# hvasbath/beat

Measured on AMD Instinct MI355X. Metric: SMC chain-steps/s (FFI seismic gfstacking 400 patches x 64 targets x 4096 samples), higher is better.
Workload: dtype f64; 1 GPU; BASELINE configs[2]: FFI seismic gfstacking, 400 patches x 64 targets x 4096 samples, library (64,400,3,25,4096) f64 = 62.9 GB in HBM, nearest_neighbor, covariance scalar; population SURVEY 8(d): nucleation U over the 20x20 fault, time 0; chains_per_gpu=512, global_chains=512, parallelism=chains sharded over 1 GPU(s), library replicated

## Files before the change

### beat_amd/_lib.py

```python
import ctypes as C
import os

import numpy as np

_HERE = os.path.dirname(os.path.abspath(__file__))
LIB_PATH = os.environ.get("BEATAMD_LIB") or os.path.join(_HERE, "libbeat_amd.so")

NEAREST_NEIGHBOR, MULTILINEAR = 0, 1
W_SCALAR, W_DENSE = 0, 1
INTERPOLATIONS = {"nearest_neighbor": NEAREST_NEIGHBOR, "multilinear": MULTILINEAR}

OK, EINVAL, EHIP, EINDEX, ENOMEM, ENAN, ENOTPSD, EBADCOV, EOUTSIDE = 0, -1, -2, -3, -4, -5, -6, -7, -8
ABI_VERSION = 120


class BeatAmdError(RuntimeError):
    pass


class FfiLayout(C.Structure):
    _fields_ = [
        ("nparams", C.c_int64),
        ("nvar", C.c_int32),
        ("slip_off", C.c_int64 * 4),
# ... 33 lines not shown
    "beatamd_geo_stack_all_batch": [_vp, _i32, _i64, _vp, _i32, _vp],
    "beatamd_weights_create": [_vp, _i32, _i64, _i64, _vp, _vp, _pi32],
    "beatamd_weights_update": [_vp, _i32, _i32, _i64, _vp, _vp],
    "beatamd_weights_destroy": [_vp, _i32],
    "beatamd_weights_band": [_vp, _i32, _pi64],
    "beatamd_weights_band_info": [_vp, _i32, _pi64, C.POINTER(_f64)],
    "beatamd_mvn_chol_logp_batch": [_vp, _i32, _i64, _vp, _vp, _vp],
    "beatamd_laplacian_create": [_vp, _i64, _vp, _f64, _pi32],
    "beatamd_laplacian_destroy": [_vp, _i32],
    "beatamd_laplacian_logp_batch": [_vp, _i32, _i64, _i64, _vp, _vp, _vp],
    "beatamd_ffi_model_create": [_vp, C.POINTER(FfiLayout), _i32, _vp, _vp, _vp, _pi32],
    "beatamd_ffi_model_add_wavemap": [_vp, _i32, _vp, _vp, _i32, _vp, _vp, _i32],
    "beatamd_ffi_model_add_geodetic": [_vp, _i32, _vp, _vp, _vp, _i32, _vp, _vp, _vp],
    "beatamd_ffi_model_add_geodetic_geometry": [_vp, _i32, _i32, _vp, _vp, _vp, _i64, _vp, _vp, _vp, _f64,
                                                _vp, _vp, _i32, _vp, _vp, _vp],
    "beatamd_ffi_model_add_geodetic_corrections": [_vp, _i32, _i32, _vp, _vp, _vp, _vp, _vp],
    "beatamd_ffi_model_set_laplacian": [_vp, _i32, _i32],
    "beatamd_ffi_model_nllk": [_vp, _i32, _pi64],
    "beatamd_ffi_model_destroy": [_vp, _i32],
    "beatamd_ffi_logp_batch": [_vp, _i32, _i64, _vp, _vp],
    "beatamd_ffi_synthetics_batch": [_vp, _i32, _i32, _i64, _vp, _i32, _vp],
    "beatamd_ffi_astep_batch": [_vp, _i32, _i64, _vp, _vp, _vp, _vp, _vp, _vp, _vp, _f64, _vp],
    "beatamd_autocovariance_batch": [_vp, _i64, _i64, _vp, _vp, _vp],
    "beatamd_scaled_toeplitz_batch": [_vp, _i64, _i64, _vp, _vp, _vp],
    "beatamd_ffi_astep_batch_betas": [_vp, _i32, _i64, _vp, _vp, _vp, _vp, _vp, _vp, _vp, _vp, _vp],
    "beatamd_ffi_mstep_batch": [_vp, _i32, _i64, _vp, _vp, _vp, _i64, _i32, _i32, C.c_uint64, C.c_uint32, _i64,
                                _vp, _vp, _vp, _f64, _vp, _vp, _vp, _vp],
    "beatamd_ctx_last_kernel": [_vp, C.c_char_p, _i64],
    "beatamd_ctx_gf_group_stats": [_vp, _pi64, C.POINTER(_f64), _pi64, _pi64],
    "beatamd_ctx_gf_plan": [_vp, C.c_char_p, _i64, C.POINTER(_f64), _pi64],
    "beatamd_ctx_gf_tune_log": [_vp, C.c_char_p, _i64],
    "beatamd_gf_patch_ranges": [_i64, _i64, _i64, C.c_int32],
    "beatamd_seis_gflib_set_split_targets": [_vp, _i32, _i64],
    "beatamd_ctx_reload_knobs": [_vp],
    "beatamd_ctx_gf_chain_groups": [_vp, _i64, _vp, _vp, _i64, _vp],
    "beatamd_smc_calc_beta": [_vp, _i64, _vp, _i64, _f64, _f64, C.POINTER(_f64), _vp],
    "beatamd_smc_stage_weights": [_vp, _i64, _vp, _i64, _f64, _vp],
    "beatamd_smc_resample": [_vp, _i64, _vp, _f64, _vp],
    "beatamd_smc_population_factor": [_vp, _i64, _i64, _vp, _vp, _vp],
    "beatamd_proposal_draw": [_vp, _i64, _i64, _i64, _vp, C.c_uint64, C.c_uint32, _i64, _i32, _vp, _vp],
    "beatamd_proposal_draw_univariate": [_vp, _i64, _i64, _i32, _vp, C.c_uint64, C.c_uint32, _i64, _vp, _vp],
    "beatamd_gather_rows": [_vp, _i64, _i64, _vp, _i64, _vp, _vp],
    "beatamd_metropolis_tune": [_vp, _i64, _vp, _vp, _i32],
    "beatamd_ffi_model_nterm": [_vp, _i32, _pi64],
    "beatamd_ffi_llks_batch": [_vp, _i32, _i64, _vp, _vp],
    "beatamd_hyper_model_create": [_vp, _i64, _i64, _vp, _vp, _vp, _vp, _i32, _vp, _pi32],
    "beatamd_hyper_model_destroy": [_vp, _i32],
    "beatamd_hyper_logp_batch": [_vp, _i32, _i64, _vp, _vp, _vp],
    "beatamd_hyper_chain_batch": [_vp, _i32, _i64, _i64, _vp, _vp, _vp, _vp, _vp, _vp, _vp, _i32, _vp, C.c_uint64,
                                  C.c_uint32, _i64, _i32, _i32, _i32, _vp, _vp],
    "beatamd_wset_quad_batch": [_vp, _i32, _i64, _vp, _vp],
    "beatamd_ffi_obs_quads": [_vp, _i32, _vp],
    "beatamd_ffi_variance_reductions_batch": [_vp, _i32, _i64, _vp, _vp],
    "beatamd_ffi_geo_residuals_batch": [_vp, _i32, _i64, _vp, _i32, _vp],
    "beatamd_standardize_batch": [_vp, _i32, _vp, _i64, _i64, _i64, _vp, _vp, _vp],
    "beatamd_ensemble_moments_update": [_vp, _i64, _i64, _vp, _vp, _i64],
    "beatamd_ensemble_moments_finish": [_vp, _i64, _vp, _i64, _vp, _vp, _vp, _vp],
    "beatamd_trace_density_update": [_vp, _i64, _i64, _i64, _vp, _vp, _f64, _vp, _i64, _i64, _f64, _vp],
    "beatamd_like_assemble": [_vp, _i64, _i64, _i64, _vp, _vp, _vp, _i64, _i64, _i64, _i64, _i32, _vp, _vp],
    "beatamd_metropolis_propose": [_vp, _i64, _i64, _vp, _vp, _vp, _vp, _vp, _vp, _vp],
    "beatamd_metropolis_accept": [_vp, _i64, _i64, _i64, _vp, _vp, _vp, _vp, _vp, _vp, _f64, _vp, _vp],
    "beatamd_whiten_rows": [_vp, _vp, _i64, _i64, _vp],
    "beatamd_whiten_rows_batch": [_vp, _vp, _i64, _i64, _i64, _vp],
    "beatamd_chol_inverse_batch": [_vp, _i64, _i64, _vp, _vp, _vp],
    "beatamd_chol_inverse_batch_flags": [_vp, _i64, _i64, _vp, _vp, _vp, _vp],
    "beatamd_whitening_ratio_batch": [_vp, _i64, _i64, _vp, _vp, _vp],
# ... 77 lines not shown
```

### beat_amd/csrc/capi.cpp

```cpp
#include "model.hpp"

using namespace beatamd;

namespace {

template <class T>
int32_t add_obj(std::vector<std::unique_ptr<T>> &v, std::unique_ptr<T> o)
{
    for (size_t i = 0; i < v.size(); i++)
        if (!v[i]) {
            v[i] = std::move(o);
            return (int32_t)i;
        }
    v.push_back(std::move(o));
    return (int32_t)v.size() - 1;
}

template <class T>
int host_copy(beatamd_ctx *ctx, const T *p, size_t n, std::vector<T> &out)
{
    out.resize(n);
    if (n == 0) return BEATAMD_OK;
    if (is_device_ptr(p)) {
        BA_HIP(hipMemcpyAsync(out.data(), p, n * sizeof(T), hipMemcpyDeviceToHost, ctx->stream));
// ... 1148 lines not shown
    *row_bytes = (int64_t)((double)tot * ctx->gs_trep) * ctx->gs_N * 8 * ctx->gs_nvar;
    return BEATAMD_OK;
}

int beatamd_ctx_gf_plan(beatamd_ctx *ctx, char *buf, int64_t buflen, double *mean_passes, int64_t *max_passes)
{
    ENTER(ctx);
    BA_CHECK(buf && buflen > 0, BEATAMD_EINVAL, "gf_plan: bad argument");
    snprintf(buf, (size_t)buflen, "%s", ctx->gf_plan);
    if (mean_passes) *mean_passes = ctx->gs_ngtp ? 1.0 : 0.0;
    if (max_passes) *max_passes = ctx->gs_ngtp ? 1 : 0;
    if (!ctx->gs_has_passes || ctx->gs_ngtp == 0 || (!mean_passes && !max_passes)) return BEATAMD_OK;
    int64_t tot = 0, mx = 0;
    BA_TRY(gs_counters(ctx, 1, &tot, &mx));
    if (mean_passes) *mean_passes = (double)tot / (double)ctx->gs_ngtp;
    if (max_passes) *max_passes = mx;
    return BEATAMD_OK;
}

int beatamd_ctx_gf_tune_log(beatamd_ctx *ctx, char *buf, int64_t buflen)
{
    ENTER(ctx);
    BA_CHECK(buf && buflen > 0, BEATAMD_EINVAL, "gf_tune_log: bad argument");
    snprintf(buf, (size_t)buflen, "%s", ctx->gf_tune_log);
    return BEATAMD_OK;
}

int32_t beatamd_gf_patch_ranges(int64_t ntargets, int64_t npatches, int64_t nsamples, int32_t num_cu)
{
    if (ntargets <= 0 || npatches <= 0 || nsamples <= 0) return 1;
    return (int32_t)gf_patch_ranges(ntargets, npatches, nsamples, num_cu > 0 ? num_cu : 256);
}

int beatamd_ctx_gf_chain_groups(beatamd_ctx *ctx, int64_t C, const double *key0, const double *key1,
                                int64_t chains_per_group, uint32_t *members)
{
    ENTER(ctx);
    BA_CHECK(C > 0 && key0 && key1 && members && chains_per_group > 0, BEATAMD_EINVAL, "gf_chain_groups: bad argument");
    const int64_t ngroups = (C + chains_per_group - 1) / chains_per_group;
    const ChainVec key[2] = {ChainVec{key0, 1, 0}, ChainVec{key1, 1, 0}};
    const uint32_t *m = nullptr;
    BA_TRY(launch_chain_members(ctx, C, key, chains_per_group, ngroups, &m));
    BA_CHECK(m != nullptr, BEATAMD_EINVAL, "gf_chain_groups: groups of more than 8192 chains are not cut");
    BA_HIP(hipStreamSynchronize(ctx->stream));
    BA_HIP(hipMemcpy(members, m, (size_t)(ngroups * chains_per_group) * sizeof(uint32_t), hipMemcpyDeviceToHost));
    return BEATAMD_OK;
}

int beatamd_smc_calc_beta(beatamd_ctx *ctx, int64_t C, const double *likelihoods, int64_t stride,
                          double beta, double coef_variation, double *beta_new, double *weights)
{
    ENTER(ctx);
    BA_CHECK(likelihoods && beta_new && weights && C > 0 && stride > 0, BEATAMD_EINVAL,
             "smc_calc_beta: bad argument");
    Staging st(ctx);
    const double *d_l;
    double *d_w, *d_out;
    BA_TRY(st.in(likelihoods, (size_t)((C - 1) * stride + 1), &d_l));
    BA_TRY(st.out(weights, (size_t)C, &d_w));
    BA_TRY(ctx->scratch(SL_STAGE2, 8, &d_out));
    BA_TRY(launch_smc_calc_beta(ctx, C, d_l, stride, beta, coef_variation, 0, 0.0, d_out, d_w));
    double out[2];
    BA_HIP(hipMemcpyAsync(out, d_out, sizeof(out), hipMemcpyDeviceToHost, ctx->stream));
    BA_TRY(st.finish());
    BA_HIP(hipStreamSynchronize(ctx->stream));
    *beta_new = out[0];
// ... 383 lines not shown
```

### beat_amd/csrc/gfshared.hip

```cpp
#include "kernels.hpp"
#include "misfit.hpp"

namespace beatamd {

constexpr int GS_NT_MAX = 64;
constexpr int GS_NTHINT_DEFAULT = 1;
constexpr int GS_WS_DEFAULT = 1;

struct GroupTabArgs {
    int nrow, nvar, CG;
    int64_t C, T, P, DS;
    const uint32_t *rowoff;
    const double *fac;
    ChainVec slips[4];
    int ucap, ustride;
    uint32_t *urows;
    uint32_t *uent;
    int nissue;
    int windowed;
    int depth;
    uint32_t *ucount;
    uint32_t *umax;
    uint16_t *slot;
    double *w;
// ... 1237 lines not shown
{
    __shared__ uint32_t wsum[WS_CG / 64];
    const int tid = threadIdx.x;
    const int lane = tid & 63, wv = tid >> 6;
    const int64_t pos = (int64_t)blockIdx.x * WS_CG + tid;
    const uint32_t c = order ? order[pos] : (pos < C ? (uint32_t)pos : 0xffffffffu);
    const bool on = c != 0xffffffffu && (int64_t)c < C && active[c] != 0;
    const uint64_t m = __ballot(on);
    if (lane == 0) wsum[wv] = (uint32_t)__popcll(m);
    __syncthreads();
    uint32_t before = 0, total = 0;
    for (int q = 0; q < WS_CG / 64; q++) {
        const uint32_t x = wsum[q];
        if (q < wv) before += x;
        total += x;
    }
    uint32_t *o = out + (int64_t)blockIdx.x * WS_CG;
    if (on) o[before + (uint32_t)__popcll(m & ((1ull << lane) - 1ull))] = c;
    if ((uint32_t)tid >= total) o[tid] = 0xffffffffu;
}

constexpr int64_t WS_MAP_MAX = 16384;
template <int FILL, int MAP>
__global__ void __launch_bounds__(WS_CG) k_ws_tables(WsTabArgs a)
{
    extern __shared__ __attribute__((aligned(16))) uint16_t rowmap[];
    __shared__ __attribute__((aligned(16))) uint32_t vals[WS_CG];
    __shared__ __attribute__((aligned(16))) uint32_t firstv[WS_CG];
    __shared__ uint32_t lst[WS_CG];
    __shared__ uint32_t gm[WS_CG];
    __shared__ uint16_t slt[WS_CG];
    __shared__ uint8_t rk2i[WS_MAXPASS][128];
    __shared__ uint32_t wsum[WS_CG / 64 + 1];
    const int tid = threadIdx.x;
    const int lane = tid & 63, wv = tid >> 6;
    const int64_t gtp = xcd_items8(blockIdx.x, gridDim.x);
    const int64_t p = gtp % a.P;
    const int64_t gt = gtp / a.P;
    const int64_t t = gt % a.T;
    const int64_t g = gt / a.T;
    const int64_t pos_in_batch = g * WS_CG + tid;
    const uint32_t oc = a.order ? a.order[pos_in_batch] : (uint32_t)pos_in_batch;
    const bool live = pos_in_batch < a.C && oc != 0xffffffffu;
    const int64_t c = live ? (int64_t)oc : 0;
    const uint32_t v = live ? a.rowoff[(c * a.T + t) * a.P + p] : 0xffffffffu;
    double sl[4] = {0.0, 0.0, 0.0, 0.0};
    if constexpr (FILL)
        for (int iv = 0; iv < a.nvar; iv++)
            if (live) sl[iv] = a.slips[iv].base[c * a.slips[iv].stride + a.slips[iv].off + (t % a.R) * a.P + p];
    gm[tid] = 0;
    uint32_t pos = 0, U = 0;
    bool first = false;
    if constexpr (MAP) {
        const uint32_t row0 = (uint32_t)((t * a.P + p) * a.DS);
        for (int64_t i = tid; i < a.DS; i += WS_CG) rowmap[i] = 0;
        __syncthreads();
        if (live) rowmap[v - row0] = 1;
        __syncthreads();
        uint32_t run = 0;
        for (int64_t base = 0; base < a.DS; base += WS_CG) {
            const int64_t i = base + tid;
            const uint32_t f = (i < a.DS) ? rowmap[i] : 0u;
            const uint64_t m = __ballot(f != 0);
            if (lane == 0) wsum[wv] = (uint32_t)__popcll(m);
            __syncthreads();
            uint32_t before = 0, total = 0;
            for (int q = 0; q < WS_CG / 64; q++) {
                const uint32_t x = wsum[q];
                if (q < wv) before += x;
                total += x;
            }
            if (f) {
                const uint32_t ps = run + before + (uint32_t)__popcll(m & ((1ull << lane) - 1ull));
                rowmap[i] = (uint16_t)ps;
                if constexpr (FILL) lst[ps] = row0 + (uint32_t)i;
            }
            run += total;
            __syncthreads();
        }
        U = run;
        if (live) pos = rowmap[v - row0];
    } else {
        vals[tid] = v;
// ... 7 lines not shown
                first = first && !((x.x == v && k < tid) || (x.y == v && k + 1 < tid) || (x.z == v && k + 2 < tid) ||
                                   (x.w == v && k + 3 < tid));
            }
        }
        firstv[tid] = first ? v : 0xffffffffu;
        {
            const uint64_t m = __ballot(first);
            if (lane == 0) wsum[wv] = (uint32_t)__popcll(m);
        }
        __syncthreads();
        if (live) {
            const uint4 *f4 = reinterpret_cast<const uint4 *>(firstv);
            for (int k4 = 0; k4 < WS_CG / 4; k4++) {
                const uint4 x = f4[k4];
                pos += (x.x < v) + (x.y < v) + (x.z < v) + (x.w < v);
            }
        }
        for (int q = 0; q < WS_CG / 64; q++) U += wsum[q];
    }
    const int npass = U == 0 ? 1 : (int)((U + (uint32_t)a.cap - 1) / (uint32_t)a.cap);
    if constexpr (!FILL) {
        if (tid == 0) {
            a.npass[gtp] = (uint32_t)npass;
            a.utotal[gtp] = U;
        }
        return;
    }
    if (tid == 0) a.utotal[gtp] = U;
    const int per = U == 0 ? 1 : ((int)U + npass - 1) / npass;
    if constexpr (!MAP) {
        if (first) lst[pos] = v;
    }
    if (live) atomicOr(&gm[pos], 1u << (tid >> 5));
    __syncthreads();
    const int mypass = live ? (int)pos / per : -1;
    if (wv < npass) {
        const int base = wv * per;
        const int n = min(per, (int)U - base);
        if (n <= 32) {
            if (lane < n) slt[base + lane] = (uint16_t)lane;
        } else {
            const int depth = a.cap / 32;
            const int r0 = lane, r1 = lane + 64;
            const uint32_t m0 = r0 < n ? gm[base + r0] : 0u, m1 = r1 < n ? gm[base + r1] : 0u;
            const int key0 = r0 < n ? ((__popc(m0) << 8) | (255 - r0)) : -1;
            const int key1 = r1 < n ? ((__popc(m1) << 8) | (255 - r1)) : -1;
            int rank0 = 0, rank1 = 0;
            for (int j = 0; j < n; j++) {
                const int kj = (__popc(gm[base + j]) << 8) | (255 - j);
                rank0 += kj > key0;
                rank1 += kj > key1;
            }
            if (r0 < n && rank0 < 32) slt[base + r0] = (uint16_t)rank0;
            if (r1 < n && rank1 < 32) slt[base + r1] = (uint16_t)rank1;
            if (r0 < n) rk2i[wv][rank0] = (uint8_t)r0;
            if (r1 < n) rk2i[wv][rank1] = (uint8_t)r1;
            wave_lds_fence();
            uint32_t wmask = 0;
            int wcnt = 0;
            if (lane < 32) {
                wmask = gm[base + rk2i[wv][lane]];
                wcnt = 1;
            }
            for (int rk = 32; rk < n; rk++) {
                const int ridx = (int)rk2i[wv][rk];
                const uint32_t mm = gm[base + ridx];
                int cost = (lane < 32 && wcnt < depth) ? ((__popc(wmask & mm) << 12) | (wcnt << 6) | lane) : 0x7fffffff;
#pragma unroll
                for (int off = 32; off > 0; off >>= 1) cost = min(cost, __shfl_xor(cost, off, 64));
                const int w = cost & 63;
                if (lane == w) {
                    slt[base + ridx] = (uint16_t)(w + 32 * wcnt);
                    wmask |= mm;
                    wcnt++;
                }
            }
        }
    }
    __syncthreads();
    const int64_t v0 = gt * a.vmax + (a.voff ? (int64_t)a.voff[gtp] : p);
    const uint16_t myslot = live ? slt[pos] : (uint16_t)0;
    constexpr int kstr = WS_USTRIDE / WS_LW;
    for (int k = 0; k < npass; k++) {
        const int64_t vs = v0 + k;
        const int base = k * per;
        const int n = min(per, (int)U - base);
        const bool mine = mypass == k;
        a.slot[vs * WS_CG + tid] = mine ? myslot : (uint16_t)a.cap;
        for (int iv = 0; iv < a.nvar; iv++) a.w[(int64_t)iv * a.w_var_stride + vs * WS_CG + tid] = mine ? sl[iv] : 0.0;
        if (tid == 0) a.ucount[vs] = (uint32_t)n;
        if (tid < WS_USTRIDE) {
            const int j = tid;
            uint32_t *e = a.uent + ((vs * WS_LW + (j % WS_LW)) * kstr + (j / WS_LW)) * 2;
            e[0] = n > 0 ? lst[base + (j < n ? j : n - 1)] : 0u;
            e[1] = j < n ? (uint32_t)slt[base + j] : 0u;
        }
    }
}

static int pick_group(int64_t C)
{
    const int cand[4] = {512, 256, 128, 64};
    const double cost[4] = {2.55, 1.5, 1.2, 1.0};
    int best = 64;
    double bestc = 1e300;
    for (int i = 0; i < 4; i++) {
        const double c = (double)((C + cand[i] - 1) / cand[i]) * cost[i];
        if (c < bestc - 1e-12) { bestc = c; best = cand[i]; }
    }
    return best;
}

static bool shared_fit(const GfStackCall &k, int cg, bool row_passes, int *ucap_out)
{
    const SeisLib &L = *k.libs[0];
    const int nrow = k.interp == BEATAMD_MULTILINEAR ? 4 : 1;
    const int64_t DS = L.D * L.S;
    const int64_t ucap = std::min<int64_t>((int64_t)cg * nrow, DS);
    if (!row_passes) {
        if (2 * ucap * (GS_NT_MAX + 2) * 8 > 158 * 1024) return false;
        if (2 * DS * 4 + cg * 4 + 2048 > 60 * 1024) return false;
// ... 55 lines not shown
    memset(&a, 0, sizeof(a));
    *f32 = k.f32;
    for (int v = 0; v < k.nvar; v++) {
        a.G[v] = k.libs[v]->g;
        a.G32[v] = k.libs[v]->g32;
        *f32 = *f32 && a.G32[v] != nullptr;
    }
    a.nvar = k.nvar;
    a.C = k.C; a.T = L.T; a.P = L.P; a.N = L.N;
    a.Ttab = Ttab; a.rows_per_target = L.P * L.D * L.S;
    a.tslot = k.tslot;
    a.ngroups = ngroups;
    a.data = k.data; a.wscalar = k.wscalar; a.out = k.out;
    a.nthint = GfKnobs::set(kn.gs_nthint) ? (kn.gs_nthint != 0) : (GS_NTHINT_DEFAULT && ngroups == 1);
}

static int64_t gs_grid(GsArgs &a, const GfKnobs &kn)
{
    a.xcd_order = (a.ngroups > 1 && !GfKnobs::is(kn.gs_order, 0)) ? 1 : 0;
    if (GfKnobs::is(kn.gs_order, 1)) a.xcd_order = 1;
    return a.xcd_order ? ((a.T * a.ntile + 7) / 8) * 8 * a.ngroups : a.ngroups * a.T * a.ntile;
}

static void gs_record_stats(beatamd_ctx *ctx, const GfStackCall &k, int64_t GTP, int64_t Ttab, int cg, bool has_passes)
{
    ctx->gs_ngtp = GTP;
    ctx->gs_trep = (double)k.libs[0]->T / (double)Ttab;
    ctx->gs_N = k.libs[0]->N;
    ctx->gs_cg = cg;
    ctx->gs_nvar = k.nvar;
    ctx->gs_has_passes = has_passes;
}

static int launch_gfstack_ws(beatamd_ctx *ctx, const GfStackCall &k, const uint32_t *rowoff, int64_t Ttab)
{
    const GfKnobs &kn = *k.knobs;
    const SeisLib &L = *k.libs[0];
    const int64_t ngroups = (k.C + WS_CG - 1) / WS_CG;
    const int64_t GT = ngroups * Ttab, GTP = GT * L.P;
    const int64_t bound = std::min<int64_t>(WS_CG, L.D * L.S);
    const int cap = bound <= 32 ? 32 : bound <= 64 ? 64 : WS_CAP_MAX;
    const int maxpass = (int)((bound + cap - 1) / cap);
    const int64_t vmax = L.P * maxpass;

    WsTabArgs ta;
    memset(&ta, 0, sizeof(ta));
    ta.nvar = k.nvar; ta.cap = cap;
    ta.C = k.C; ta.T = Ttab; ta.P = L.P; ta.DS = L.D * L.S; ta.vmax = vmax;
    ta.rowoff = rowoff;
    for (int v = 0; v < k.nvar; v++) ta.slips[v] = k.slips[v];
    ta.R = k.patch_split;
    if (ngroups > 1 && k.order_key[0].base && k.order_key[1].base && GfKnobs::get(kn.gc_global, 1) != 0)
        BA_TRY(launch_chain_members(ctx, k.C, k.order_key, WS_CG, ngroups, &ta.order, GfKnobs::get(kn.gc_global, 1) == 2));
    BA_TRY(ctx->scratch(SL_GS_UCOUNT, (size_t)(3 * GTP + GT), &ta.utotal));
    ta.npass = ta.utotal + GTP;
    uint32_t *voff = ta.npass + GTP, *nv = voff + GTP;
    const size_t nvs = (size_t)GT * vmax + 3;
    BA_TRY(ctx->scratch(SL_GS_UROWS, nvs, &ta.ucount));
    BA_TRY(ctx->scratch(SL_GS_USLOT, nvs * WS_USTRIDE * 2, &ta.uent));
    BA_TRY(ctx->scratch(SL_GS_SLOT, nvs * WS_CG, &ta.slot));
    ta.w_var_stride = (int64_t)GT * vmax * WS_CG;
    BA_TRY(ctx->scratch(SL_GS_W, (size_t)ta.w_var_stride * k.nvar + (size_t)3 * WS_CG, &ta.w));
    {
        ScopedTimer tm(ctx, "grouptables");
        if (k.active) {
            uint32_t *packed;
            BA_TRY(ctx->scratch(SL_WS_PACK, (size_t)ngroups * WS_CG, &packed));
            hipLaunchKernelGGL(k_ws_pack, dim3((unsigned)ngroups), dim3(WS_CG), 0, ctx->stream, ta.order, k.active, k.C, packed);
            ta.order = packed;
        }
        const bool map = ta.DS <= WS_MAP_MAX && !GfKnobs::is(kn.ws_map, 0);
        const size_t mlds = map ? (size_t)ta.DS * sizeof(uint16_t) : 0;
        if (maxpass > 1) {
            if (map) hipLaunchKernelGGL((k_ws_tables<0, 1>), dim3((unsigned)GTP), dim3(WS_CG), mlds, ctx->stream, ta);
            else hipLaunchKernelGGL((k_ws_tables<0, 0>), dim3((unsigned)GTP), dim3(WS_CG), 0, ctx->stream, ta);
            hipLaunchKernelGGL(k_ws_scan, dim3((unsigned)GT), dim3(256), 0, ctx->stream, ta.npass, voff, nv, L.P);
            ta.voff = voff;
        }
        if (map) hipLaunchKernelGGL((k_ws_tables<1, 1>), dim3((unsigned)GTP), dim3(WS_CG), mlds, ctx->stream, ta);
        else hipLaunchKernelGGL((k_ws_tables<1, 0>), dim3((unsigned)GTP), dim3(WS_CG), 0, ctx->stream, ta);
    }
    BA_HIP(hipGetLastError());

    GsArgs a;
    bool f32;
    gs_common_args(a, k, Ttab, ngroups, &f32);
    const bool pair64 = GfKnobs::is(kn.gs_pair, 1);
    a.nrow = 1;
    a.CG = WS_CG; a.ucap = cap; a.ustride = WS_USTRIDE;
    a.nt = 64; a.dma = 2; a.ws = 3;
    a.ntile = (int)((L.N + 63) / 64);
    a.nv = maxpass > 1 ? nv : nullptr;
    a.vmax = vmax;
    a.order = ta.order;
    a.uent = ta.uent; a.ucount = ta.ucount; a.slot = ta.slot; a.w = ta.w;
    a.w_var_stride = ta.w_var_stride;
    if (k.mode == GF_RESID_SCALAR || k.mode == GF_RESID_BAND1) {
        BA_TRY(ctx->scratch(SL_PARTIAL, (size_t)k.C * L.T * a.ntile, &a.partial));
    }
    if (k.mode == GF_RESID_BAND1) {
        BA_TRY(ctx->scratch(SL_EDGES, (size_t)k.C * L.T * a.ntile * 2, &a.edges));
        a.band_w = k.band_w;
    }
    const int64_t nblocks = gs_grid(a, kn);
    BA_CHECK(nblocks < (int64_t)0x7fffffff, BEATAMD_EINVAL, "gfstack: batch too large");
    size_t lds = f32 ? (size_t)(cap + 1) * (64 + 2) * sizeof(float) * 3
                     : (size_t)(cap + 1) * (64 + (pair64 ? 2 : 1)) * sizeof(double) * 3;
    lds = std::max<size_t>(lds, (64 + 8 * 64 * 17) * sizeof(double));
    BA_CHECK(lds <= 160 * 1024, BEATAMD_EINVAL, "internal: k_gfstack_ws row buffers exceed LDS");
    if (f32 || pair64)
        snprintf(ctx->last_gf_kernel, sizeof(ctx->last_gf_kernel), "k_gfstack_ws%s<%d,%d,%d>", f32 ? "32" : "p64", k.mode, a.ws,
                 a.nthint);
    else
        snprintf(ctx->last_gf_kernel, sizeof(ctx->last_gf_kernel), "k_gfstack_ws<%d,%d,%d,%d>", 1, k.mode, a.ws, a.nthint);
    snprintf(ctx->gf_plan, sizeof(ctx->gf_plan),
             "loader/consumer kernel: 512-chain groups, nearest neighbour; %d row slots per LDS buffer (a patch can touch min(512, "
             "D*S = %lld) rows), %s", cap, (long long)(L.D * L.S),
             maxpass > 1 ? "patches that touch more are staged in passes of equal size" : "one pass per patch");
    gs_record_stats(ctx, k, GTP, Ttab, WS_CG, maxpass > 1);
    {
        ScopedTimer tm(ctx, "gfstack");
        BA_TRY(launch_ws(k.mode, dim3((unsigned)nblocks), lds, ctx->stream, a, f32 ? 1 : (pair64 ? 2 : 0)));
    }
    BA_HIP(hipGetLastError());
    if (a.partial)
// ... 151 lines not shown
```

### beat_amd/csrc/kernels.hpp

```cpp
#pragma once
#include <algorithm>

#include "ctx.hpp"

namespace beatamd {

int launch_sweep_explicit(beatamd_ctx *ctx, const double *slow, double h, const int32_t *hi,
                          const int32_t *hj, int ni, int nj, int64_t C, double *out);
int launch_sweep_model(beatamd_ctx *ctx, const FfiModel &m, const double *Q, int64_t C,
                       double *starttimes0, int32_t *chain_bad);

struct StartTimeSrc {
    const double *explicit_st = nullptr;
    const double *starttimes0 = nullptr;
    const double *Q = nullptr;
    int64_t nparams = 0;
    const int64_t *shift_off = nullptr;
    int32_t nslot = 0;
    const int32_t *tslot = nullptr;
    const int64_t *slot_shift_off = nullptr;
    int32_t *chain_bad = nullptr;
};

struct ChainVec {
// ... 24 lines not shown
{
    return by != GF_BY_OTHER && !GfKnobs::is(kn.qf_fuse, 0);
}

struct GfStackCall {
    const SeisLib *libs[4] = {nullptr, nullptr, nullptr, nullptr};
    int nvar = 1;
    ChainVec slips[4];
    ChainVec durations;
    StartTimeSrc st;
    int interp = 0;
    int64_t C = 0;
    int mode = GF_STORE_SYN;
    const double *data = nullptr;
    const double *wscalar = nullptr;
    double *out = nullptr;
    double *quad = nullptr;
    const double *band_w = nullptr;
    bool f32 = false;
    ChainVec order_key[2];
    int patch_split = 1;
    const GfKnobs *knobs = nullptr;
    const int32_t *tslot = nullptr;
    const int32_t *active = nullptr;
};
int launch_gfstack(beatamd_ctx *ctx, const GfStackCall &call);
int launch_sum_tiles(beatamd_ctx *ctx, const double *partial, int64_t n, int ntile, double *quad, const int *guard = nullptr,
                     int want = 0, const double *edges = nullptr, const double *band_w = nullptr, int64_t T = 1, int64_t N = 0);
int launch_round_to_f32(beatamd_ctx *ctx, double *g, float *g32, int64_t n);
bool gfstack_shared_applicable(const GfStackCall &call, int *cg, int *ucap);
int gfstack_shared_candidates(const GfStackCall &call, int *cgs, int *ucaps);
int launch_gfstack_shared(beatamd_ctx *ctx, const GfStackCall &call, const uint32_t *rowoff,
                          const double *fac, int CG, int ucap, int64_t Ttab, bool *band1_done);

int launch_chain_members(beatamd_ctx *ctx, int64_t C, const ChainVec key[2], int64_t cg, int64_t ngroups, const uint32_t **members,
                         int strips = 0);
bool gfstack_ml_applicable(const GfStackCall &call);
int launch_gfstack_ml(beatamd_ctx *ctx, const GfStackCall &call, const uint32_t *rowoff,
                      const double *fac, int64_t Ttab, const int **ovf);

struct QuadformCall {
    const double *A = nullptr;
    int64_t a_stride = 0;
    int64_t M = 0, nd = 0, C = 0;
    const double *X = nullptr;
    int64_t xs_c = 0, xs_d = 0;
    int upper_tri = 0;
    double *quad = nullptr;
    int64_t q_stride = 0;
};
int launch_quadform(beatamd_ctx *ctx, const QuadformCall &call);
constexpr int QF_BAND_LIMIT = 16;
int launch_band_detect(beatamd_ctx *ctx, const double *A, int64_t nd, int64_t M, void *scratch, int64_t *band_host,
                       double *dropped_rel_host);
int launch_band_pack(beatamd_ctx *ctx, const double *A, int64_t nd, int64_t M, int64_t band, double *wb);
int launch_quadform_banded(beatamd_ctx *ctx, const double *wb, int64_t band, int64_t M, int64_t nd, int64_t C, const double *X,
                           int64_t xs_c, int64_t xs_d, double *quad, int64_t q_stride, const int *guard = nullptr, int want = 0);
struct QuadformSmallCall {
    int nd = 0;
    const double *A[8];
    int64_t M[8], xoff[8];
    int upper_tri[8];
    const double *slog[8];
    const int64_t *hp_off[8];
    int64_t C = 0;
    const double *X = nullptr;
// ... 182 lines not shown
```

### beat_amd/engine.py

```python
import ctypes as C

import numpy as np

from . import _lib
from ._lib import INTERPOLATIONS, check, f64, ptr


def _is_dev(a):
    return hasattr(a, "data_ptr") and not isinstance(a, np.ndarray) and a.is_cuda


def _empty_like(ref, shape, dtype=np.float64):
    if _is_dev(ref):
        import torch
        tdt = {np.float64: torch.float64, np.int32: torch.int32}[dtype]
        return torch.empty(shape, dtype=tdt, device=ref.device)
    return np.empty(shape, dtype=dtype)


def _i32(a, ref=None):
    if _is_dev(a):
        import torch
        if a.dtype != torch.int32 or not a.is_contiguous():
            raise ValueError("device index tensors must be contiguous int32")
# ... 384 lines not shown
                    row_bytes=rb.value)

    def reload_knobs(self):
        check(self._lib.beatamd_ctx_reload_knobs(self._h))

    def gf_plan(self, passes=True):
        buf = C.create_string_buffer(512)
        mean, mx = C.c_double(), C.c_int64()
        check(self._lib.beatamd_ctx_gf_plan(self._h, buf, 512, C.byref(mean) if passes else None,
                                            C.byref(mx) if passes else None))
        out = dict(plan=buf.value.decode())
        if passes:
            out.update(mean_passes=mean.value, max_passes=mx.value)
        return out

    def gf_tune_log(self):
        buf = C.create_string_buffer(512)
        check(self._lib.beatamd_ctx_gf_tune_log(self._h, buf, 512))
        return buf.value.decode()

    def gf_chain_groups(self, key0, key1, chains_per_group=512):
        import torch
        dev = "cuda:%d" % self.device
        k0, k1 = [k if _is_dev(k) else torch.as_tensor(np.ascontiguousarray(k, dtype=np.float64)).to(dev) for k in (key0, key1)]
        self._adopt_stream(k0, k1)
        k0, k1 = f64(k0), f64(k1)
        Cn = int(k0.numel())
        ng = (Cn + chains_per_group - 1) // chains_per_group
        out = np.empty(ng * chains_per_group, dtype=np.uint32)
        check(self._lib.beatamd_ctx_gf_chain_groups(self._h, Cn, ptr(k0), ptr(k1), int(chains_per_group),
                                                    out.ctypes.data_as(C.c_void_p)))
        return out.reshape(ng, chains_per_group)

    def smc_calc_beta(self, likelihoods, beta, coef_variation, stride=1, n=None):
        self._adopt_stream(likelihoods)
        lk = f64(likelihoods)
        Cn = int(n if n is not None else (lk.numel() if _is_dev(lk) else lk.size))
        w = _empty_like(lk, (Cn,))
        b = C.c_double()
        check(self._lib.beatamd_smc_calc_beta(self._h, Cn, ptr(lk), int(stride), float(beta),
                                              float(coef_variation), C.byref(b), ptr(w)))
        return b.value, w

    def smc_stage_weights(self, likelihoods, dbeta, stride=1, n=None):
        self._adopt_stream(likelihoods)
        lk = f64(likelihoods)
        Cn = int(n if n is not None else (lk.numel() if _is_dev(lk) else lk.size))
        w = _empty_like(lk, (Cn,))
        check(self._lib.beatamd_smc_stage_weights(self._h, Cn, ptr(lk), int(stride), float(dbeta), ptr(w)))
        return w

    def smc_resample(self, weights, aux):
        self._adopt_stream(weights)
        w = f64(weights)
        Cn = int(w.numel()) if _is_dev(w) else int(w.size)
        idx = _empty_like(w, (Cn,), np.int32)
        check(self._lib.beatamd_smc_resample(self._h, Cn, ptr(w), float(aux), ptr(idx)))
        return idx

    def smc_population_factor(self, population, weights):
        self._adopt_stream(population, weights)
        X, w = f64(population), f64(weights)
        Cn, npar = int(X.shape[0]), int(X.shape[1])
        F = _empty_like(X, (Cn, npar))
        check(self._lib.beatamd_smc_population_factor(self._h, Cn, npar, ptr(X), ptr(w), ptr(F)))
        return F
# ... 345 lines not shown
```

### include/beat_amd.h

```cpp
#ifndef BEAT_AMD_H
#define BEAT_AMD_H

#include <stdint.h>

#ifdef __cplusplus
extern "C" {
#endif

#define BEATAMD_OK 0
#define BEATAMD_EINVAL (-1)
#define BEATAMD_EHIP (-2)
#define BEATAMD_EINDEX (-3)
#define BEATAMD_ENOMEM (-4)
#define BEATAMD_ENAN (-5)
#define BEATAMD_ENOTPSD (-6)
#define BEATAMD_EOUTSIDE (-8)
#define BEATAMD_EBADCOV (-7)

#define BEATAMD_VERSION 120

#define BEATAMD_NEAREST_NEIGHBOR 0
#define BEATAMD_MULTILINEAR 1

#define BEATAMD_W_SCALAR 0
#define BEATAMD_W_DENSE 1

typedef struct beatamd_ctx beatamd_ctx;

const char *beatamd_last_error(void);
int beatamd_version(void);

int beatamd_ctx_create(int device, beatamd_ctx **out);
int beatamd_ctx_destroy(beatamd_ctx *ctx);
int beatamd_ctx_set_stream(beatamd_ctx *ctx, void *hip_stream);
int beatamd_ctx_use_own_stream(beatamd_ctx *ctx);
int beatamd_ctx_synchronize(beatamd_ctx *ctx);
int beatamd_ctx_reload_knobs(beatamd_ctx *ctx);
int beatamd_ctx_set_step_counter(beatamd_ctx *ctx, uint32_t *device_counter);
int beatamd_ctx_enable_timing(beatamd_ctx *ctx, int on);
int beatamd_ctx_kernel_time(beatamd_ctx *ctx, const char *kernel, double *total_ms,
                            int64_t *launches);
int beatamd_ctx_reset_timing(beatamd_ctx *ctx);
int beatamd_ctx_last_kernel(beatamd_ctx *ctx, char *buf, int64_t buflen);
int beatamd_ctx_gf_group_stats(beatamd_ctx *ctx, int64_t *chains_per_group, double *mean_rows,
                               int64_t *max_rows, int64_t *row_bytes);
int beatamd_ctx_gf_plan(beatamd_ctx *ctx, char *buf, int64_t buflen, double *mean_passes, int64_t *max_passes);
int beatamd_ctx_gf_tune_log(beatamd_ctx *ctx, char *buf, int64_t buflen);
int32_t beatamd_gf_patch_ranges(int64_t ntargets, int64_t npatches, int64_t nsamples, int32_t num_cu);
int beatamd_seis_gflib_set_split_targets(beatamd_ctx *ctx, int32_t lib_id, int64_t ntargets);

int beatamd_ctx_gf_chain_groups(beatamd_ctx *ctx, int64_t C, const double *key0, const double *key1,
                                int64_t chains_per_group, uint32_t *members);

int beatamd_fast_sweep_batch(beatamd_ctx *ctx, const double *slowness, double patch_size,
                             const int32_t *h_strk, const int32_t *h_dip, int32_t num_strk,
                             int32_t num_dip, int64_t C, double *out);

int beatamd_seis_gflib_create(beatamd_ctx *ctx, int64_t ntargets, int64_t npatches,
                              int64_t ndurations, int64_t nstarttimes, int64_t nsamples,
                              double starttime_min, double starttime_sampling,
                              double duration_min, double duration_sampling, int32_t *lib_id);
int beatamd_seis_gflib_upload(beatamd_ctx *ctx, int32_t lib_id, const double *src,
                              int64_t offset, int64_t count);
int beatamd_seis_gflib_adopt(beatamd_ctx *ctx, int32_t lib_id, double *device_ptr);
int beatamd_seis_gflib_round_to_f32(beatamd_ctx *ctx, int32_t lib_id);
int beatamd_ffi_model_set_f32(beatamd_ctx *ctx, int32_t model_id, int32_t wavemap_index, int32_t on);
int beatamd_seis_gflib_device_ptr(beatamd_ctx *ctx, int32_t lib_id, double **device_ptr);
int beatamd_seis_gflib_destroy(beatamd_ctx *ctx, int32_t lib_id);

int beatamd_seis_stack_all_batch(beatamd_ctx *ctx, int32_t lib_id, int64_t C,
                                 const double *durations, const double *starttimes,
                                 const double *slips, int32_t interpolation, double *out);

int beatamd_geo_gflib_create(beatamd_ctx *ctx, int64_t npatches, int64_t nobs, const double *G,
                             int32_t *lib_id);
int beatamd_geo_gflib_destroy(beatamd_ctx *ctx, int32_t lib_id);
int beatamd_geo_stack_all_batch(beatamd_ctx *ctx, int32_t lib_id, int64_t C,
                                const double *slips, int32_t accumulate, double *out);

int beatamd_weights_create(beatamd_ctx *ctx, int32_t kind, int64_t ndatasets, int64_t M,
                           const double *weights, const double *slog_pdet, int32_t *wset_id);
int beatamd_weights_update(beatamd_ctx *ctx, int32_t wset_id, int32_t kind, int64_t count,
// ... 164 lines not shown
```

Baseline: 89740 chain-steps/s.

## Let idle half-waves alias live lanes' slots and refine pass slot assignment

In the work-set table kernel, each pass now records which half-waves contain live chains not belonging to that pass. The fast identity slot assignment is used only when no such foreign half-waves exist; otherwise every row goes through the greedy cost-based assignment, seeded with those half-wave masks. Non-live lanes now copy the slot of a live lane in their half-wave instead of pointing at the empty cap slot, which should cut the number of distinct rows touched per half-wave in the gather. It also adds a host-callable API that exposes the table builder for inspection, plus some refactoring, at the cost of extra ballots and atomics during table construction.

Result: no change. 89610 chain-steps/s (-0.1%).

```diff
diff --git a/beat_amd/_lib.py b/beat_amd/_lib.py
--- a/beat_amd/_lib.py
+++ b/beat_amd/_lib.py
@@ -89,6 +89,7 @@
     "beatamd_ctx_gf_tune_log": [_vp, C.c_char_p, _i64],
     "beatamd_gf_patch_ranges": [_i64, _i64, _i64, C.c_int32],
     "beatamd_seis_gflib_set_split_targets": [_vp, _i32, _i64],
+    "beatamd_gf_ws_tables": [_vp, _i64, _i64, _i64, _i64, _vp, _vp, _pi64, _pi64, _vp, _vp, _vp, _vp, _vp, _vp, _vp],
     "beatamd_ctx_reload_knobs": [_vp],
     "beatamd_ctx_gf_chain_groups": [_vp, _i64, _vp, _vp, _i64, _vp],
     "beatamd_smc_calc_beta": [_vp, _i64, _vp, _i64, _f64, _f64, C.POINTER(_f64), _vp],
diff --git a/beat_amd/csrc/capi.cpp b/beat_amd/csrc/capi.cpp
--- a/beat_amd/csrc/capi.cpp
+++ b/beat_amd/csrc/capi.cpp
@@ -1204,6 +1204,28 @@
     return (int32_t)gf_patch_ranges(ntargets, npatches, nsamples, num_cu > 0 ? num_cu : 256);
 }
 
+int beatamd_gf_ws_tables(beatamd_ctx *ctx, int64_t C, int64_t T, int64_t P, int64_t DS, const uint32_t *row_ids,
+                         const int32_t *active, int64_t *cap, int64_t *vmax, uint32_t *order, uint32_t *nv, uint32_t *voff,
+                         uint32_t *ucount, uint32_t *uent, uint16_t *slot, double *w)
+{
+    ENTER(ctx);
+    BA_CHECK(C > 0 && T > 0 && P > 0 && DS > 0 && cap && vmax, BEATAMD_EINVAL, "gf_ws_tables: bad argument");
+    BA_CHECK(C * T * P < (int64_t)1 << 31 && T * P * DS < (int64_t)1 << 32, BEATAMD_EINVAL, "gf_ws_tables: too large");
+    if (!row_ids) return ws_tables_to_host(ctx, C, T, P, DS, nullptr, nullptr, cap, vmax, order, nv, voff, ucount, uent, slot, w);
+    BA_CHECK(!is_device_ptr(row_ids) && !(active && is_device_ptr(active)), BEATAMD_EINVAL, "gf_ws_tables: host arrays expected");
+    for (int64_t c = 0; c < C; c++)
+        for (int64_t tp = 0; tp < T * P; tp++) {
+            const int64_t r = (int64_t)row_ids[c * T * P + tp] - tp * DS;
+            BA_CHECK(r >= 0 && r < DS, BEATAMD_EINDEX, "gf_ws_tables: row id outside the rows of its (target, patch)");
+        }
+    Staging st(ctx);
+    const uint32_t *d_rows;
+    const int32_t *d_act;
+    BA_TRY(st.in(row_ids, (size_t)(C * T * P), &d_rows));
+    BA_TRY(st.in(active, (size_t)C, &d_act));
+    return ws_tables_to_host(ctx, C, T, P, DS, d_rows, d_act, cap, vmax, order, nv, voff, ucount, uent, slot, w);
+}
+
 int beatamd_ctx_gf_chain_groups(beatamd_ctx *ctx, int64_t C, const double *key0, const double *key1,
                                 int64_t chains_per_group, uint32_t *members)
 {
diff --git a/beat_amd/csrc/gfshared.hip b/beat_amd/csrc/gfshared.hip
--- a/beat_amd/csrc/gfshared.hip
+++ b/beat_amd/csrc/gfshared.hip
@@ -1293,6 +1293,7 @@
     __shared__ uint16_t slt[WS_CG];
     __shared__ uint8_t rk2i[WS_MAXPASS][128];
     __shared__ uint32_t wsum[WS_CG / 64 + 1];
+    __shared__ uint32_t zgrp[WS_MAXPASS];
     const int tid = threadIdx.x;
     const int lane = tid & 63, wv = tid >> 6;
     const int64_t gtp = xcd_items8(blockIdx.x, gridDim.x);
@@ -1310,6 +1311,8 @@
         for (int iv = 0; iv < a.nvar; iv++)
             if (live) sl[iv] = a.slips[iv].base[c * a.slips[iv].stride + a.slips[iv].off + (t % a.R) * a.P + p];
     gm[tid] = 0;
+    if constexpr (FILL)
+        if (tid < WS_MAXPASS) zgrp[tid] = 0;
     uint32_t pos = 0, U = 0;
     bool first = false;
     if constexpr (MAP) {
@@ -1383,12 +1386,18 @@
         if (first) lst[pos] = v;
     }
     if (live) atomicOr(&gm[pos], 1u << (tid >> 5));
+    const int mypass = live ? (int)pos / per : -1;
+    for (int k = 0; k < npass && npass > 1; k++) {
+        const uint64_t m = __ballot(live && mypass != k);
+        const uint32_t two = (uint32_t)((m & 0xffffffffull) != 0) | ((uint32_t)((m >> 32) != 0) << 1);
+        if (lane == 0 && two) atomicOr(&zgrp[k], two << (2 * wv));
+    }
     __syncthreads();
-    const int mypass = live ? (int)pos / per : -1;
     if (wv < npass) {
         const int base = wv * per;
         const int n = min(per, (int)U - base);
-        if (n <= 32) {
+        const uint32_t z = zgrp[wv];
+        if (n <= 32 && z == 0) {
             if (lane < n) slt[base + lane] = (uint16_t)lane;
         } else {
             const int depth = a.cap / 32;
@@ -1402,18 +1411,19 @@
                 rank0 += kj > key0;
                 rank1 += kj > key1;
             }
-            if (r0 < n && rank0 < 32) slt[base + r0] = (uint16_t)rank0;
-            if (r1 < n && rank1 < 32) slt[base + r1] = (uint16_t)rank1;
+            const int pre = z == 0 ? 32 : 0;
+            if (r0 < n && rank0 < pre) slt[base + r0] = (uint16_t)rank0;
+            if (r1 < n && rank1 < pre) slt[base + r1] = (uint16_t)rank1;
             if (r0 < n) rk2i[wv][rank0] = (uint8_t)r0;
             if (r1 < n) rk2i[wv][rank1] = (uint8_t)r1;
             wave_lds_fence();
-            uint32_t wmask = 0;
+            uint32_t wmask = lane == a.cap % 32 ? z : 0u;
             int wcnt = 0;
-            if (lane < 32) {
+            if (lane < pre) {
                 wmask = gm[base + rk2i[wv][lane]];
                 wcnt = 1;
             }
-            for (int rk = 32; rk < n; rk++) {
+            for (int rk = pre; rk < n; rk++) {
                 const int ridx = (int)rk2i[wv][rk];
                 const uint32_t mm = gm[base + ridx];
                 int cost = (lane < 32 && wcnt < depth) ? ((__popc(wmask & mm) << 12) | (wcnt << 6) | lane) : 0x7fffffff;
@@ -1431,13 +1441,18 @@
     __syncthreads();
     const int64_t v0 = gt * a.vmax + (a.voff ? (int64_t)a.voff[gtp] : p);
     const uint16_t myslot = live ? slt[pos] : (uint16_t)0;
+    const uint64_t livem = __ballot(live);
+    const uint32_t liveh = (uint32_t)(livem >> (lane & 32));
+    const int alias = liveh ? (lane & 32) + __ffs(liveh) - 1 : lane;
     constexpr int kstr = WS_USTRIDE / WS_LW;
     for (int k = 0; k < npass; k++) {
         const int64_t vs = v0 + k;
         const int base = k * per;
         const int n = min(per, (int)U - base);
         const bool mine = mypass == k;
-        a.slot[vs * WS_CG + tid] = mine ? myslot : (uint16_t)a.cap;
+        const int sk = mine ? (int)myslot : a.cap;
+        const int sa = __shfl(sk, alias, 64);
+        a.slot[vs * WS_CG + tid] = (uint16_t)(live ? sk : sa);
         for (int iv = 0; iv < a.nvar; iv++) a.w[(int64_t)iv * a.w_var_stride + vs * WS_CG + tid] = mine ? sl[iv] : 0.0;
         if (tid == 0) a.ucount[vs] = (uint32_t)n;
         if (tid < WS_USTRIDE) {
@@ -1559,55 +1574,127 @@
     ctx->gs_has_passes = has_passes;
 }
 
+struct WsGeom {
+    int64_t ngroups, vmax;
+    int cap, maxpass;
+};
+static WsGeom ws_geometry(int64_t C, int64_t P, int64_t DS)
+{
+    WsGeom g;
+    g.ngroups = (C + WS_CG - 1) / WS_CG;
+    const int64_t bound = std::min<int64_t>(WS_CG, DS);
+    g.cap = bound <= 32 ? 32 : bound <= 64 ? 64 : WS_CAP_MAX;
+    g.maxpass = (int)((bound + g.cap - 1) / g.cap);
+    g.vmax = P * g.maxpass;
+    return g;
+}
+
+static int ws_build_tables(beatamd_ctx *ctx, WsTabArgs &ta, const int32_t *active, const GfKnobs &kn, const WsGeom &g,
+                           const uint32_t **nv_out)
+{
+    const int64_t GT = g.ngroups * ta.T, GTP = GT * ta.P;
+    ta.cap = g.cap;
+    ta.vmax = g.vmax;
+    BA_TRY(ctx->scratch(SL_GS_UCOUNT, (size_t)(3 * GTP + GT), &ta.utotal));
+    ta.npass = ta.utotal + GTP;
+    uint32_t *voff = ta.npass + GTP, *nv = voff + GTP;
+    const size_t nvs = (size_t)GT * g.vmax + 3;
+    BA_TRY(ctx->scratch(SL_GS_UROWS, nvs, &ta.ucount));
+    BA_TRY(ctx->scratch(SL_GS_USLOT, nvs * WS_USTRIDE * 2, &ta.uent));
+    BA_TRY(ctx->scratch(SL_GS_SLOT, nvs * WS_CG, &ta.slot));
+    ta.w_var_stride = (int64_t)GT * g.vmax * WS_CG;
+    BA_TRY(ctx->scratch(SL_GS_W, (size_t)ta.w_var_stride * ta.nvar + (size_t)3 * WS_CG, &ta.w));
+    *nv_out = nullptr;
+    {
+        ScopedTimer tm(ctx, "grouptables");
+        if (active) {
+            uint32_t *packed;
+            BA_TRY(ctx->scratch(SL_WS_PACK, (size_t)g.ngroups * WS_CG, &packed));
+            hipLaunchKernelGGL(k_ws_pack, dim3((unsigned)g.ngroups), dim3(WS_CG), 0, ctx->stream, ta.order, active, ta.C, packed);
+            ta.order = packed;
+        }
+        const bool map = ta.DS <= WS_MAP_MAX && !GfKnobs::is(kn.ws_map, 0);
+        const size_t mlds = map ? (size_t)ta.DS * sizeof(uint16_t) : 0;
+        if (g.maxpass > 1) {
+            if (map) hipLaunchKernelGGL((k_ws_tables<0, 1>), dim3((unsigned)GTP), dim3(WS_CG), mlds, ctx->stream, ta);
+            else hipLaunchKernelGGL((k_ws_tables<0, 0>), dim3((unsigned)GTP), dim3(WS_CG), 0, ctx->stream, ta);
+            hipLaunchKernelGGL(k_ws_scan, dim3((unsigned)GT), dim3(256), 0, ctx->stream, ta.npass, voff, nv, ta.P);
+            ta.voff = voff;
+            *nv_out = nv;
+        }
+        if (map) hipLaunchKernelGGL((k_ws_tables<1, 1>), dim3((unsigned)GTP), dim3(WS_CG), mlds, ctx->stream, ta);
+        else hipLaunchKernelGGL((k_ws_tables<1, 0>), dim3((unsigned)GTP), dim3(WS_CG), 0, ctx->stream, ta);
+    }
+    BA_HIP(hipGetLastError());
+    return BEATAMD_OK;
+}
+
+int ws_tables_to_host(beatamd_ctx *ctx, int64_t C, int64_t T, int64_t P, int64_t DS, const uint32_t *rowoff, const int32_t *active,
+                      int64_t *cap, int64_t *vmax, uint32_t *order, uint32_t *nv, uint32_t *voff, uint32_t *ucount, uint32_t *uent,
+                      uint16_t *slot, double *w)
+{
+    const WsGeom g = ws_geometry(C, P, DS);
+    *cap = g.cap;
+    *vmax = g.vmax;
+    if (!rowoff) return BEATAMD_OK;
+    const int64_t GT = g.ngroups * T;
+    std::vector<double> ones((size_t)P, 1.0);
+    double *d_ones;
+    BA_TRY(ctx->scratch(SL_SLIPS, (size_t)P, &d_ones));
+    BA_HIP(hipMemcpyAsync(d_ones, ones.data(), (size_t)P * sizeof(double), hipMemcpyHostToDevice, ctx->stream));
+    WsTabArgs ta;
+    memset(&ta, 0, sizeof(ta));
+    ta.nvar = 1;
+    ta.C = C; ta.T = T; ta.P = P; ta.DS = DS;
+    ta.rowoff = rowoff;
+    ta.slips[0] = ChainVec{d_ones, 0, 0};
+    ta.R = 1;
+    const uint32_t *d_nv;
+    BA_TRY(ws_build_tables(ctx, ta, active, gf_knobs(ctx), g, &d_nv));
+    const auto back = [&](void *host, const void *dev, size_t bytes) {
+        return host ? hipMemcpyAsync(host, dev, bytes, hipMemcpyDeviceToHost, ctx->stream) : hipSuccess;
+    };
+    const size_t nvs = (size_t)GT * g.vmax;
+    if (ta.order) BA_HIP(back(order, ta.order, (size_t)g.ngroups * WS_CG * sizeof(uint32_t)));
+    if (d_nv) {
+        BA_HIP(back(nv, d_nv, (size_t)GT * sizeof(uint32_t)));
+        BA_HIP(back(voff, ta.voff, (size_t)GT * P * sizeof(uint32_t)));
+    }
+    BA_HIP(back(ucount, ta.ucount, nvs * sizeof(uint32_t)));
+    BA_HIP(back(uent, ta.uent, nvs * WS_USTRIDE * 2 * sizeof(uint32_t)));
+    BA_HIP(back(slot, ta.slot, nvs * WS_CG * sizeof(uint16_t)));
+    BA_HIP(back(w, ta.w, nvs * WS_CG * sizeof(double)));
+    BA_TRY(ctx->check_status());
+    if (!ta.order && order)
+        for (int64_t i = 0; i < g.ngroups * WS_CG; i++) order[i] = i < C ? (uint32_t)i : 0xffffffffu;
+    if (!d_nv)
+        for (int64_t gt = 0; gt < GT; gt++) {
+            if (nv) nv[gt] = (uint32_t)P;
+            for (int64_t p = 0; p < P && voff; p++) voff[gt * P + p] = (uint32_t)p;
+        }
+    return BEATAMD_OK;
+}
+
 static int launch_gfstack_ws(beatamd_ctx *ctx, const GfStackCall &k, const uint32_t *rowoff, int64_t Ttab)
 {
     const GfKnobs &kn = *k.knobs;
     const SeisLib &L = *k.libs[0];
-    const int64_t ngroups = (k.C + WS_CG - 1) / WS_CG;
-    const int64_t GT = ngroups * Ttab, GTP = GT * L.P;
-    const int64_t bound = std::min<int64_t>(WS_CG, L.D * L.S);
-    const int cap = bound <= 32 ? 32 : bound <= 64 ? 64 : WS_CAP_MAX;
-    const int maxpass = (int)((bound + cap - 1) / cap);
-    const int64_t vmax = L.P * maxpass;
+    const WsGeom geom = ws_geometry(k.C, L.P, L.D * L.S);
+    const int64_t ngroups = geom.ngroups, vmax = geom.vmax;
+    const int cap = geom.cap, maxpass = geom.maxpass;
+    const int64_t GTP = ngroups * Ttab * L.P;
 
     WsTabArgs ta;
     memset(&ta, 0, sizeof(ta));
-    ta.nvar = k.nvar; ta.cap = cap;
-    ta.C = k.C; ta.T = Ttab; ta.P = L.P; ta.DS = L.D * L.S; ta.vmax = vmax;
+    ta.nvar = k.nvar;
+    ta.C = k.C; ta.T = Ttab; ta.P = L.P; ta.DS = L.D * L.S;
     ta.rowoff = rowoff;
     for (int v = 0; v < k.nvar; v++) ta.slips[v] = k.slips[v];
     ta.R = k.patch_split;
     if (ngroups > 1 && k.order_key[0].base && k.order_key[1].base && GfKnobs::get(kn.gc_global, 1) != 0)
         BA_TRY(launch_chain_members(ctx, k.C, k.order_key, WS_CG, ngroups, &ta.order, GfKnobs::get(kn.gc_global, 1) == 2));
-    BA_TRY(ctx->scratch(SL_GS_UCOUNT, (size_t)(3 * GTP + GT), &ta.utotal));
-    ta.npass = ta.utotal + GTP;
-    uint32_t *voff = ta.npass + GTP, *nv = voff + GTP;
-    const size_t nvs = (size_t)GT * vmax + 3;
-    BA_TRY(ctx->scratch(SL_GS_UROWS, nvs, &ta.ucount));
-    BA_TRY(ctx->scratch(SL_GS_USLOT, nvs * WS_USTRIDE * 2, &ta.uent));
-    BA_TRY(ctx->scratch(SL_GS_SLOT, nvs * WS_CG, &ta.slot));
-    ta.w_var_stride = (int64_t)GT * vmax * WS_CG;
-    BA_TRY(ctx->scratch(SL_GS_W, (size_t)ta.w_var_stride * k.nvar + (size_t)3 * WS_CG, &ta.w));
-    {
-        ScopedTimer tm(ctx, "grouptables");
-        if (k.active) {
-            uint32_t *packed;
-            BA_TRY(ctx->scratch(SL_WS_PACK, (size_t)ngroups * WS_CG, &packed));
-            hipLaunchKernelGGL(k_ws_pack, dim3((unsigned)ngroups), dim3(WS_CG), 0, ctx->stream, ta.order, k.active, k.C, packed);
-            ta.order = packed;
-        }
-        const bool map = ta.DS <= WS_MAP_MAX && !GfKnobs::is(kn.ws_map, 0);
-        const size_t mlds = map ? (size_t)ta.DS * sizeof(uint16_t) : 0;
-        if (maxpass > 1) {
-            if (map) hipLaunchKernelGGL((k_ws_tables<0, 1>), dim3((unsigned)GTP), dim3(WS_CG), mlds, ctx->stream, ta);
-            else hipLaunchKernelGGL((k_ws_tables<0, 0>), dim3((unsigned)GTP), dim3(WS_CG), 0, ctx->stream, ta);
-            hipLaunchKernelGGL(k_ws_scan, dim3((unsigned)GT), dim3(256), 0, ctx->stream, ta.npass, voff, nv, L.P);
-            ta.voff = voff;
-        }
-        if (map) hipLaunchKernelGGL((k_ws_tables<1, 1>), dim3((unsigned)GTP), dim3(WS_CG), mlds, ctx->stream, ta);
-        else hipLaunchKernelGGL((k_ws_tables<1, 0>), dim3((unsigned)GTP), dim3(WS_CG), 0, ctx->stream, ta);
-    }
-    BA_HIP(hipGetLastError());
+    const uint32_t *nv;
+    BA_TRY(ws_build_tables(ctx, ta, k.active, kn, geom, &nv));
 
     GsArgs a;
     bool f32;
@@ -1617,7 +1704,7 @@
     a.CG = WS_CG; a.ucap = cap; a.ustride = WS_USTRIDE;
     a.nt = 64; a.dma = 2; a.ws = 3;
     a.ntile = (int)((L.N + 63) / 64);
-    a.nv = maxpass > 1 ? nv : nullptr;
+    a.nv = nv;
     a.vmax = vmax;
     a.order = ta.order;
     a.uent = ta.uent; a.ucount = ta.ucount; a.slot = ta.slot; a.w = ta.w;
diff --git a/beat_amd/csrc/kernels.hpp b/beat_amd/csrc/kernels.hpp
--- a/beat_amd/csrc/kernels.hpp
+++ b/beat_amd/csrc/kernels.hpp
@@ -80,6 +80,9 @@
 int gfstack_shared_candidates(const GfStackCall &call, int *cgs, int *ucaps);
 int launch_gfstack_shared(beatamd_ctx *ctx, const GfStackCall &call, const uint32_t *rowoff,
                           const double *fac, int CG, int ucap, int64_t Ttab, bool *band1_done);
+int ws_tables_to_host(beatamd_ctx *ctx, int64_t C, int64_t T, int64_t P, int64_t DS, const uint32_t *rowoff, const int32_t *active,
+                      int64_t *cap, int64_t *vmax, uint32_t *order, uint32_t *nv, uint32_t *voff, uint32_t *ucount, uint32_t *uent,
+                      uint16_t *slot, double *w);
 
 int launch_chain_members(beatamd_ctx *ctx, int64_t C, const ChainVec key[2], int64_t cg, int64_t ngroups, const uint32_t **members,
                          int strips = 0);
diff --git a/beat_amd/engine.py b/beat_amd/engine.py
--- a/beat_amd/engine.py
+++ b/beat_amd/engine.py
@@ -440,6 +440,25 @@
                                                     out.ctypes.data_as(C.c_void_p)))
         return out.reshape(ng, chains_per_group)
 
+    def gf_ws_tables(self, row_ids, DS, active=None):
+        rows = np.ascontiguousarray(row_ids, dtype=np.uint32)
+        Cn, T, P = rows.shape
+        act = None if active is None else np.ascontiguousarray(active, dtype=np.int32)
+        if act is not None and act.shape != (Cn,):
+            raise ValueError("active must have one entry per chain")
+        cap, vmax = C.c_int64(), C.c_int64()
+        nul = [None] * 7
+        check(self._lib.beatamd_gf_ws_tables(self._h, Cn, T, P, int(DS), None, None, C.byref(cap), C.byref(vmax), *nul))
+        G, V = (Cn + 511) // 512, vmax.value
+        out = dict(order=np.full((G, 512), 0xffffffff, np.uint32), nv=np.zeros((G, T), np.uint32),
+                   voff=np.zeros((G, T, P), np.uint32), ucount=np.zeros((G, T, V), np.uint32),
+                   uent=np.zeros((G, T, V, 4, 32, 2), np.uint32), slot=np.zeros((G, T, V, 512), np.uint16),
+                   w=np.zeros((G, T, V, 512), np.float64))
+        check(self._lib.beatamd_gf_ws_tables(self._h, Cn, T, P, int(DS), ptr(rows), ptr(act), C.byref(cap), C.byref(vmax),
+                                             *[ptr(out[k]) for k in ("order", "nv", "voff", "ucount", "uent", "slot", "w")]))
+        out["cap"] = cap.value
+        return out
+
     def smc_calc_beta(self, likelihoods, beta, coef_variation, stride=1, n=None):
         self._adopt_stream(likelihoods)
         lk = f64(likelihoods)
diff --git a/include/beat_amd.h b/include/beat_amd.h
--- a/include/beat_amd.h
+++ b/include/beat_amd.h
@@ -48,6 +48,9 @@
 int beatamd_ctx_gf_tune_log(beatamd_ctx *ctx, char *buf, int64_t buflen);
 int32_t beatamd_gf_patch_ranges(int64_t ntargets, int64_t npatches, int64_t nsamples, int32_t num_cu);
 int beatamd_seis_gflib_set_split_targets(beatamd_ctx *ctx, int32_t lib_id, int64_t ntargets);
+int beatamd_gf_ws_tables(beatamd_ctx *ctx, int64_t C, int64_t T, int64_t P, int64_t DS, const uint32_t *row_ids,
+                         const int32_t *active, int64_t *cap, int64_t *vmax, uint32_t *order, uint32_t *nv, uint32_t *voff,
+                         uint32_t *ucount, uint32_t *uent, uint16_t *slot, double *w);
 
 int beatamd_ctx_gf_chain_groups(beatamd_ctx *ctx, int64_t C, const double *key0, const double *key1,
                                 int64_t chains_per_group, uint32_t *members);
```
